# rafaelsoStanford/State_Policy_DiffusionModel

Hardware: AMD Instinct MI355X
Metric: denoise-steps/sec (B=4096, horizon=32) (higher is better)
Workload: dtype f32 (split-fp16 MFMA operands, fp32 accumulate)

## Files before the change

state_policy_diffusionmodel_amd/csrc/device_utils.h:

```cpp
#pragma once
#include <hip/hip_runtime.h>
#include "kernels.h"

namespace spdm {

__device__ __forceinline__ void sample_mean_rstd(const StatsRef& st, int b, float& mean, float& rstd) {
    const long long r0 = (long long)b * st.HW;
    const int first = (int)(r0 / st.m_tile);
    const int last = (int)((r0 + st.HW - 1) / st.m_tile);
    const int n = (last - first + 1) * st.n_tiles;
    const double* p = st.p + (size_t)b * st.slots * 2;
    double s1 = 0.0, s2 = 0.0;
    for (int i = 0; i < n; ++i) { s1 += p[2 * i]; s2 += p[2 * i + 1]; }
    const double m = s1 * st.inv_count;
    double var = s2 * st.inv_count - m * m;
    if (var < 0.0) var = 0.0;
    mean = (float)m;
    rstd = (float)(1.0 / sqrt(var + 1e-5));
}

__device__ __forceinline__ float sum_xor32(float v) {
    const unsigned u = __builtin_bit_cast(unsigned, v);
    const auto r = __builtin_amdgcn_permlane32_swap(u, u, false, false);
    return __builtin_bit_cast(float, (unsigned)r[0]) + __builtin_bit_cast(float, (unsigned)r[1]);
}
__device__ __forceinline__ float max_xor32(float v) {
    const unsigned u = __builtin_bit_cast(unsigned, v);
    const auto r = __builtin_amdgcn_permlane32_swap(u, u, false, false);
    return fmaxf(__builtin_bit_cast(float, (unsigned)r[0]), __builtin_bit_cast(float, (unsigned)r[1]));
}
__device__ __forceinline__ float sum_xor16(float v) {
    const unsigned u = __builtin_bit_cast(unsigned, v);
    const auto r = __builtin_amdgcn_permlane16_swap(u, u, false, false);
    return __builtin_bit_cast(float, (unsigned)r[0]) + __builtin_bit_cast(float, (unsigned)r[1]);
}
__device__ __forceinline__ double sum_xor32_f64(double v) {
    const unsigned long long u = __builtin_bit_cast(unsigned long long, v);
    const unsigned lo = (unsigned)u, hi = (unsigned)(u >> 32);
    const auto rl = __builtin_amdgcn_permlane32_swap(lo, lo, false, false);
    const auto rh = __builtin_amdgcn_permlane32_swap(hi, hi, false, false);
    const double a = __builtin_bit_cast(double, ((unsigned long long)(unsigned)rh[0] << 32) | (unsigned)rl[0]);
    const double b = __builtin_bit_cast(double, ((unsigned long long)(unsigned)rh[1] << 32) | (unsigned)rl[1]);
    return a + b;
}
__device__ __forceinline__ double sum_xor16_f64(double v) {
    const unsigned long long u = __builtin_bit_cast(unsigned long long, v);
    const unsigned lo = (unsigned)u, hi = (unsigned)(u >> 32);
    const auto rl = __builtin_amdgcn_permlane16_swap(lo, lo, false, false);
    const auto rh = __builtin_amdgcn_permlane16_swap(hi, hi, false, false);
    const double a = __builtin_bit_cast(double, ((unsigned long long)(unsigned)rh[0] << 32) | (unsigned)rl[0]);
    const double b = __builtin_bit_cast(double, ((unsigned long long)(unsigned)rh[1] << 32) | (unsigned)rl[1]);
    return a + b;
}

__device__ __forceinline__ void split_pair_f16(float a, float b, unsigned& hi, unsigned& lo) {
    unsigned h;
    float la, lb;
    asm("v_cvt_pk_f16_f32 %0, %1, %2" : "=v"(h) : "v"(a), "v"(b));
    asm("v_fma_mix_f32 %0, %1, -1.0, %2 op_sel:[0,0,0] op_sel_hi:[1,0,0]" : "=v"(la) : "v"(h), "v"(a));
    asm("v_fma_mix_f32 %0, %1, -1.0, %2 op_sel:[1,0,0] op_sel_hi:[1,0,0]" : "=v"(lb) : "v"(h), "v"(b));
    asm("v_cvt_pk_f16_f32 %0, %1, %2" : "=v"(lo) : "v"(la), "v"(lb));
    hi = h;
}

__device__ __forceinline__ double wave_sum_f64(double v) {
#define DPP_ADD64(ctrl_)                                                                                        \
    {                                                                                                           \
        const unsigned long long u_ = __builtin_bit_cast(unsigned long long, v);                                \
        const int lo_ = __builtin_amdgcn_update_dpp(0, (int)(unsigned)u_, ctrl_, 0xf, 0xf, false);             \
        const int hi_ = __builtin_amdgcn_update_dpp(0, (int)(unsigned)(u_ >> 32), ctrl_, 0xf, 0xf, false);     \
        v += __builtin_bit_cast(double, ((unsigned long long)(unsigned)hi_ << 32) | (unsigned long long)(unsigned)lo_); \
    }
    DPP_ADD64(0xB1)
    DPP_ADD64(0x4E)
    DPP_ADD64(0x141)
    DPP_ADD64(0x140)
#undef DPP_ADD64
    v = sum_xor16_f64(v);
    v = sum_xor32_f64(v);
    return v;
}

__device__ __forceinline__ double seg_sum_f64(double v, int seg) {
#define DPP_ADD64(ctrl_)                                                                                        \
    {                                                                                                           \
        const unsigned long long u_ = __builtin_bit_cast(unsigned long long, v);                                \
        const int lo_ = __builtin_amdgcn_update_dpp(0, (int)(unsigned)u_, ctrl_, 0xf, 0xf, false);             \
        const int hi_ = __builtin_amdgcn_update_dpp(0, (int)(unsigned)(u_ >> 32), ctrl_, 0xf, 0xf, false);     \
        v += __builtin_bit_cast(double, ((unsigned long long)(unsigned)hi_ << 32) | (unsigned long long)(unsigned)lo_); \
    }
    if (seg > 1) DPP_ADD64(0xB1)
    if (seg > 2) DPP_ADD64(0x4E)
    if (seg > 4) DPP_ADD64(0x141)
    if (seg > 8) DPP_ADD64(0x140)
#undef DPP_ADD64
    if (seg > 16) v = sum_xor16_f64(v);
    if (seg > 32) v = sum_xor32_f64(v);
    return v;
}

__device__ __forceinline__ void sample_mean_rstd_wave(const StatsRef& st, int b, int lane, float& mean, float& rstd) {
    const long long r0 = (long long)b * st.HW;
    const int first = (int)(r0 / st.m_tile);
    const int last = (int)((r0 + st.HW - 1) / st.m_tile);
    const int n = (last - first + 1) * st.n_tiles;
    if (n <= 8) {
        sample_mean_rstd(st, b, mean, rstd);
        return;
    }
    const double* p = st.p + (size_t)b * st.slots * 2;
    double s1 = 0.0, s2 = 0.0;
// ... 86 lines not shown
```

state_policy_diffusionmodel_amd/csrc/sa_tail.hip:

```cpp
#include <algorithm>
#include <cstdlib>

#include "device_utils.h"

namespace spdm {

namespace {

typedef float tf32x4 __attribute__((ext_vector_type(4)));
typedef float tf32x2 __attribute__((ext_vector_type(2)));
typedef _Float16 tf16x8 __attribute__((ext_vector_type(8)));
typedef _Float16 tf16x2 __attribute__((ext_vector_type(2)));

constexpr float T_ACT_SCALE = 16.0f;
constexpr float T_DESCALE = 1.0f / 2048.0f;
constexpr int T_LDK = 36;
template <int C> struct TailShape {
    static_assert(C == 128 || C == 256, "C = 128 or 256");
    static constexpr int TM = 8192 / C;
    static constexpr int WM = TM / 32, WN = 4 / WM;
    static constexpr int NCH = C / 32;
    static constexpr int TPR = C / 4, RPP = 256 / TPR;
    static constexpr int NP = TM / RPP;
};

struct SaTailArgs {
    const float* o;
    const float* x;
    float* out;
    int M;
    const float *wf_o, *wf_1, *wf_2;
    const float *b_o, *b_1, *b_2, *ln_g, *ln_b;
    const float* ab; int L;
    FilmSpec fs;
};

__device__ __forceinline__ tf32x2 tsplit2_plain(float a, float b) {
    const float xa = a * T_ACT_SCALE, xb = b * T_ACT_SCALE;
    const _Float16 ha = (_Float16)xa, hb = (_Float16)xb;
    const tf16x2 h = {ha, hb};
    const tf16x2 l = {(_Float16)(xa - (float)ha), (_Float16)(xb - (float)hb)};
    return tf32x2{__builtin_bit_cast(float, h), __builtin_bit_cast(float, l)};
}
#define TAIL_SPLIT2 tsplit2
__device__ __forceinline__ tf32x2 tsplit2(float a, float b) {
    unsigned h, l;
    split_pair_f16(a * T_ACT_SCALE, b * T_ACT_SCALE, h, l);
    return tf32x2{__builtin_bit_cast(float, h), __builtin_bit_cast(float, l)};
}
template <int TPR>
__device__ __forceinline__ float trow_sum(float v) {
    static_assert(TPR == 32 || TPR == 64, "rows of 32 or 64 lanes");
    v = sum_xor16(row16_sum_dpp(v));
    if (TPR == 64) v = sum_xor32(v);
    return v;
}

template <int C>
__device__ __forceinline__ void tail_film_fold(tf32x4 (&v)[8], const float* __restrict__ ab, int L, int m0, int M, int cq, int srow0) {
    using S = TailShape<C>;
    if (L % S::TM == 0) {
        const float* ab_ = ab + (size_t)(m0 / L) * 2 * C + cq * 4;
        const tf32x4 A = *reinterpret_cast<const tf32x4*>(ab_), B = *reinterpret_cast<const tf32x4*>(ab_ + C);
#pragma unroll
        for (int i = 0; i < 8; ++i) v[i] = v[i] * A + B;
    } else {
#pragma unroll
        for (int i = 0; i < 8; ++i) {
            const float* ab_ = ab + (size_t)(min(m0 + S::RPP * i + srow0, M - 1) / L) * 2 * C + cq * 4;
            v[i] = v[i] * *reinterpret_cast<const tf32x4*>(ab_) + *reinterpret_cast<const tf32x4*>(ab_ + C);
        }
    }
}

template <int C>
__device__ __forceinline__ void tail_film_rows(const FilmSpec& fs, int L, int m0, int M, int wave, int lane, float* abl) {
    using S = TailShape<C>;
    const int b_first = m0 / L, b_last = (min(m0 + S::TM, M) - 1) / L;
    for (int sidx = wave; sidx <= b_last - b_first; sidx += 4) film_coef_row_wave(fs, b_first + sidx, lane, abl + (size_t)sidx * 2 * C);
}
template <int C>
__device__ __forceinline__ void tail_film_fold_lds(tf32x4 (&v)[8], const float* abl, int L, int m0, int M, int cq, int srow0) {
    using S = TailShape<C>;
    const int b_first = m0 / L;
    if (L % S::TM == 0) {
        const tf32x4 A = *reinterpret_cast<const tf32x4*>(abl + cq * 4), B = *reinterpret_cast<const tf32x4*>(abl + C + cq * 4);
#pragma unroll
        for (int i = 0; i < 8; ++i) v[i] = v[i] * A + B;
    } else {
#pragma unroll
        for (int i = 0; i < 8; ++i) {
            const float* ab_ = abl + (size_t)(min(m0 + S::RPP * i + srow0, M - 1) / L - b_first) * 2 * C + cq * 4;
            v[i] = v[i] * *reinterpret_cast<const tf32x4*>(ab_) + *reinterpret_cast<const tf32x4*>(ab_ + C);
        }
    }
}

#ifdef SPDM_DIAG_TAIL
__device__ unsigned long long g_tail_stamps[64];
#define TAIL_STAMP(k_) if (blockIdx.x == 0 && threadIdx.x == 0) { asm volatile("s_waitcnt vmcnt(0) lgkmcnt(0)" ::: "memory"); g_tail_stamps[(C == 256 ? 16 : 0) + (k_)] = __builtin_amdgcn_s_memrealtime(); }
#else
#define TAIL_STAMP(k_)
#endif

template <int C>
__global__ __launch_bounds__(256, 2) void sa_tail_kernel(const SaTailArgs a) {
    TAIL_STAMP(0)
    using S = TailShape<C>;
    constexpr int T_C = C, T_M = S::TM, NCH = S::NCH, RPP = S::RPP, TPR = S::TPR;
    constexpr int RT = 2, CT = 4;
    constexpr int NP = S::NP;
    extern __shared__ __attribute__((aligned(16))) float smem[];
    const int tid = threadIdx.x, lane = tid & 63;
    const int wave = __builtin_amdgcn_readfirstlane(tid >> 6);
    const int wm = wave / S::WN, wn = wave % S::WN, l16 = lane & 15, kg = lane >> 4;
    const int M = a.M;
    const int m0 = blockIdx.x * T_M;

    float* Abuf = smem;
    float* otile = smem;

    const int c16 = tid % TPR, srow0 = tid / TPR;
    const int aoff0 = (wm * 32 + l16) * T_LDK + kg * 4;

    const size_t wlane = ((size_t)(wn * CT) * 2) * 256 + lane * 4;
    constexpr size_t WCHUNK = (size_t)(C / 16) * 2 * 256;
    tf16x8 fb[2][CT][2], fa[2][2];
#define TAIL_LOAD_B(slot_, w_, kc_)                                                                  \
    {                                                                                                \
        const float* p_ = (w_) + wlane + (size_t)(kc_) * WCHUNK;                                     \
        _Pragma("unroll") for (int c_ = 0; c_ < CT; ++c_) {                                         \
            fb[slot_][c_][0] = *reinterpret_cast<const tf16x8*>(p_ + c_ * 512);                      \
            fb[slot_][c_][1] = *reinterpret_cast<const tf16x8*>(p_ + c_ * 512 + 256);                \
        }                                                                                            \
    }
#define TAIL_LOAD_FA(slot_, kc_, rt_)                                                                \
    {                                                                                                \
        const float* p_ = Abuf + ((kc_) * T_M + (rt_) * 16) * T_LDK + aoff0;                         \
        fa[slot_][0] = *reinterpret_cast<const tf16x8*>(p_);                                         \
        fa[slot_][1] = *reinterpret_cast<const tf16x8*>(p_ + 16);                                    \
    }
#define TAIL_WRITE_SLAB(v_)                                                                          \
    _Pragma("unroll") for (int i_ = 0; i_ < NP; ++i_) {                                             \
        const tf32x2 p0_ = TAIL_SPLIT2(v_[i_].x, v_[i_].y), p1_ = TAIL_SPLIT2(v_[i_].z, v_[i_].w);   \
        float* rowp_ = Abuf + ((c16 >> 3) * T_M + RPP * i_ + srow0) * T_LDK;                         \
        *reinterpret_cast<tf32x2*>(rowp_ + (c16 & 7) * 2) = tf32x2{p0_.x, p1_.x};                    \
        *reinterpret_cast<tf32x2*>(rowp_ + 16 + (c16 & 7) * 2) = tf32x2{p0_.y, p1_.y};               \
    }
#define TAIL_GEMM(w_, wnext_)                                                                        \
    {                                                                                                \
        _Pragma("unroll") for (int rt_ = 0; rt_ < RT; ++rt_)                                        \
            _Pragma("unroll") for (int ct_ = 0; ct_ < CT; ++ct_) acc[rt_][ct_] = tf32x4{0.f, 0.f, 0.f, 0.f}; \
        TAIL_LOAD_FA(0, 0, 0)                                                                        \
        _Pragma("unroll") for (int kc = 0; kc < NCH; ++kc) {                                        \
            if (kc + 1 < NCH) { TAIL_LOAD_B((kc + 1) & 1, w_, kc + 1) } else { TAIL_LOAD_B(0, wnext_, 0) } \
            _Pragma("unroll") for (int rt = 0; rt < RT; ++rt) {                                     \
                if (rt + 1 < RT) { TAIL_LOAD_FA((rt + 1) & 1, kc, rt + 1) }                          \
                else if (kc + 1 < NCH) { TAIL_LOAD_FA(0, kc + 1, 0) }                                \
                __builtin_amdgcn_sched_barrier(0);                                                   \
                _Pragma("unroll") for (int c = 0; c < CT; ++c)                                      \
                    acc[rt][c] = __builtin_amdgcn_mfma_f32_16x16x32_f16(fa[rt & 1][0], fb[kc & 1][c][0], acc[rt][c], 0, 0, 0); \
                _Pragma("unroll") for (int c = 0; c < CT; ++c)                                      \
                    acc[rt][c] = __builtin_amdgcn_mfma_f32_16x16x32_f16(fa[rt & 1][0], fb[kc & 1][c][1], acc[rt][c], 0, 0, 0); \
                _Pragma("unroll") for (int c = 0; c < CT; ++c)                                      \
                    acc[rt][c] = __builtin_amdgcn_mfma_f32_16x16x32_f16(fa[rt & 1][1], fb[kc & 1][c][0], acc[rt][c], 0, 0, 0); \
                __builtin_amdgcn_sched_barrier(0);                                                   \
            }                                                                                        \
        }                                                                                            \
    }
#define TAIL_ACC_TO_TILE()                                                                           \
    {                                                                                                \
        __syncthreads();                                                                             \
        _Pragma("unroll") for (int rt_ = 0; rt_ < RT; ++rt_)                                        \
            _Pragma("unroll") for (int ct_ = 0; ct_ < CT; ++ct_) {                                  \
                const int col_ = wn * 64 + ct_ * 16 + l16;                                           \
                _Pragma("unroll") for (int j_ = 0; j_ < 4; ++j_)                                    \
                    otile[(wm * 32 + rt_ * 16 + 4 * kg + j_) * T_C + col_] = acc[rt_][ct_][j_] * T_DESCALE; \
            }                                                                                        \
        __syncthreads();                                                                             \
    }

    TAIL_LOAD_B(0, a.wf_o, 0)
    float* abl = smem + NCH * T_M * T_LDK;
    const tf32x4 bo = *reinterpret_cast<const tf32x4*>(a.b_o + c16 * 4);
    const tf32x4 g4 = *reinterpret_cast<const tf32x4*>(a.ln_g + c16 * 4);
// ... 150 lines not shown
        if (a.ab != nullptr) tail_film_fold<C>(v, a.ab, a.L, m0, M, c16, srow0);
        if (a.fs.on) {
            float* abl = smem + NCH * T_M * T_LDK;
            tail_film_rows<C>(a.fs, a.L, m0, M, wave, lane, abl);
            __syncthreads();
            tail_film_fold_lds<C>(v, abl, a.L, m0, M, c16, srow0);
        }
        float part[NP];
#pragma unroll
        for (int i = 0; i < NP; ++i) part[i] = (v[i].x + v[i].y) + (v[i].z + v[i].w);
#pragma unroll
        for (int i = 0; i < NP; ++i) part[i] = row16_sum_dpp(part[i]);
#pragma unroll
        for (int i = 0; i < NP; ++i) part[i] = sum_xor16(part[i]);
        if (TPR == 64) {
#pragma unroll
            for (int i = 0; i < NP; ++i) part[i] = sum_xor32(part[i]);
        }
#pragma unroll
        for (int i = 0; i < NP; ++i) {
            const float mean = part[i] * (1.0f / (float)C);
            const tf32x4 t = v[i];
            const tf32x4 d = {t.x - mean, t.y - mean, t.z - mean, t.w - mean};
            v[i] = d;
            part[i] = (d.x * d.x + d.y * d.y) + (d.z * d.z + d.w * d.w);
        }
#pragma unroll
        for (int i = 0; i < NP; ++i) part[i] = row16_sum_dpp(part[i]);
#pragma unroll
        for (int i = 0; i < NP; ++i) part[i] = sum_xor16(part[i]);
        if (TPR == 64) {
#pragma unroll
            for (int i = 0; i < NP; ++i) part[i] = sum_xor32(part[i]);
        }
#pragma unroll
        for (int i = 0; i < NP; ++i) {
            const float rstd = __builtin_amdgcn_rsqf(part[i] * (1.0f / (float)C) + 1e-5f);
            const tf32x4 d = v[i];
            v[i] = tf32x4{d.x * rstd * g4.x + b4.x, d.y * rstd * g4.y + b4.y, d.z * rstd * g4.z + b4.z, d.w * rstd * g4.w + b4.w};
        }
    }
    TAIL_WRITE_SLAB(v)
    __syncthreads();
    for (int g = g_lo; g < g_hi; ++g) {
        const float* wg = a.wf + (size_t)g * WPROD;
        const float* wnext = a.wf + (size_t)(g < 2 ? g + 1 : g) * WPROD;
        const tf32x4 bi = *reinterpret_cast<const tf32x4*>(a.b_in + g * T_C + c16 * 4);
        TAIL_GEMM(wg, wnext)
        {
            float* ot = smem + NCH * T_M * T_LDK;
            if (g > g_lo) __syncthreads();
#pragma unroll
            for (int rt_ = 0; rt_ < RT; ++rt_)
#pragma unroll
                for (int ct_ = 0; ct_ < CT; ++ct_) {
                    const int col_ = wn * 64 + ct_ * 16 + l16;
#pragma unroll
                    for (int j_ = 0; j_ < 4; ++j_)
                        ot[(wm * 32 + rt_ * 16 + 4 * kg + j_) * T_C + col_] = acc[rt_][ct_][j_] * T_DESCALE;
                }
            __syncthreads();
#pragma unroll
            for (int i = 0; i < NP; ++i) {
                const int r = RPP * i + srow0;
                if (m0 + r < M) {
                    tf32x4 t = *reinterpret_cast<const tf32x4*>(ot + r * T_C + c16 * 4);
                    t += bi;
                    *reinterpret_cast<tf32x4*>(a.qkv + (size_t)(m0 + r) * (3 * T_C) + g * T_C + c16 * 4) = t;
                }
            }
        }
    }
    (void)otile;
}

struct SaHeadArgs {
    const float* x; float* att; int M;
    const float* wf;
    const float *b_in, *ln_g, *ln_b;
    const float* ab; int L;
    FilmSpec fs;
};

__device__ __forceinline__ float row16_max_dpp(float v) {
#define DPP_MAX(ctrl_) v = fmaxf(v, __builtin_bit_cast(float, __builtin_amdgcn_update_dpp(0, __builtin_bit_cast(int, v), ctrl_, 0xf, 0xf, false)));
    DPP_MAX(0xB1) DPP_MAX(0x4E) DPP_MAX(0x141) DPP_MAX(0x140)
#undef DPP_MAX
    return v;
}
__device__ __forceinline__ float head_exp_neg(float x) {
    const float t = x * 1.44269504f;
    const float tl = __fmaf_rn(x, 1.44269504f, -t) + x * 1.925963033e-8f;
    return __builtin_amdgcn_exp2f(t) * (1.0f + tl * 0.69314718f);
}

#undef TAIL_SPLIT2
#define TAIL_SPLIT2 tsplit2_plain
template <int C>
__global__ __launch_bounds__(256, 2) void sa_head_kernel(const SaHeadArgs a) {
    using S = TailShape<C>;
    constexpr int T_C = C, T_M = S::TM, NCH = S::NCH, RPP = S::RPP, TPR = S::TPR;
    constexpr int NP = S::NP;
    constexpr int D = C / 4;
    constexpr int QROW = 2 * D + 8;
    constexpr int VROW = 2 * T_M + 8;
    constexpr int NKT = T_M / 16;
    constexpr int NDT = D / 16;
    static_assert(T_M * VROW <= 2 * T_M * QROW, "P aliases the q / k tiles");
    extern __shared__ __attribute__((aligned(16))) float smem[];
    const int tid = threadIdx.x, lane = tid & 63;
    const int wave = __builtin_amdgcn_readfirstlane(tid >> 6);
    const int l16 = lane & 15, kg = lane >> 4;
    const int M = a.M, L = a.L;
    const int m0 = blockIdx.x * T_M;
    float* Abuf = smem;
    _Float16* Qs = reinterpret_cast<_Float16*>(smem + NCH * T_M * T_LDK);
    _Float16* Ks = Qs + T_M * QROW;
    _Float16* Vt = Ks + T_M * QROW;
    _Float16* Ps = Qs;
    const int c16 = tid % TPR, srow0 = tid / TPR;

    {
        tf32x4 v[NP];
        const tf32x4 g4 = *reinterpret_cast<const tf32x4*>(a.ln_g + c16 * 4);
        const tf32x4 b4 = *reinterpret_cast<const tf32x4*>(a.ln_b + c16 * 4);
#pragma unroll
        for (int i = 0; i < NP; ++i) {
            const int row = min(m0 + RPP * i + srow0, M - 1);
            v[i] = *reinterpret_cast<const tf32x4*>(a.x + (size_t)row * T_C + c16 * 4);
        }
        if (a.ab != nullptr) tail_film_fold<C>(v, a.ab, a.L, m0, M, c16, srow0);
        if (a.fs.on) {
            float* abl = reinterpret_cast<float*>(Qs);
            tail_film_rows<C>(a.fs, a.L, m0, M, wave, lane, abl);
            __syncthreads();
            tail_film_fold_lds<C>(v, abl, a.L, m0, M, c16, srow0);
            __syncthreads();
        }
        float part[NP];
#pragma unroll
        for (int i = 0; i < NP; ++i) part[i] = (v[i].x + v[i].y) + (v[i].z + v[i].w);
#pragma unroll
        for (int i = 0; i < NP; ++i) part[i] = trow_sum<TPR>(part[i]);
#pragma unroll
        for (int i = 0; i < NP; ++i) {
            const float mean = part[i] * (1.0f / (float)C);
            const tf32x4 t = v[i];
            const tf32x4 d = {t.x - mean, t.y - mean, t.z - mean, t.w - mean};
            v[i] = d;
            part[i] = (d.x * d.x + d.y * d.y) + (d.z * d.z + d.w * d.w);
        }
#pragma unroll
        for (int i = 0; i < NP; ++i) part[i] = trow_sum<TPR>(part[i]);
#pragma unroll
        for (int i = 0; i < NP; ++i) {
            const float rstd = __builtin_amdgcn_rsqf(part[i] * (1.0f / (float)C) + 1e-5f);
            const tf32x4 d = v[i];
            v[i] = tf32x4{d.x * rstd * g4.x + b4.x, d.y * rstd * g4.y + b4.y, d.z * rstd * g4.z + b4.z, d.w * rstd * g4.w + b4.w};
        }
        TAIL_WRITE_SLAB(v)
    }
    __syncthreads();

    const int rtw = (C == 128) ? wave : (wave >> 1);
    const int cpw = (C == 128) ? 0 : (wave & 1);
    const bool attn_wave = wave < NKT;
    const float qscale = (D == 32) ? 0.17677669529663687f : 0.125f;
    constexpr size_t WCHUNK = (size_t)(3 * C / 16) * 2 * 256;

    tf16x8 fbw[2][2][2];
#define HEAD_WPTR(h_, g_) (a.wf + ((size_t)((g_) * (C / 16) + (h_) * (D / 16) + cpw * 2) * 2) * 256 + lane * 4)
#define HEAD_LOAD_W(slot_, wp_, kc_)                                                                 \
    _Pragma("unroll") for (int ct_ = 0; ct_ < 2; ++ct_) {                                           \
        fbw[slot_][ct_][0] = *reinterpret_cast<const tf16x8*>((wp_) + (size_t)(kc_) * WCHUNK + ct_ * 512);        \
        fbw[slot_][ct_][1] = *reinterpret_cast<const tf16x8*>((wp_) + (size_t)(kc_) * WCHUNK + ct_ * 512 + 256);  \
    }
    HEAD_LOAD_W(0, HEAD_WPTR(0, 0), 0)
    for (int h = 0; h < 4; ++h) {
#pragma unroll
        for (int g = 0; g < 3; ++g) {
            tf32x4 acc[2] = {tf32x4{0.f, 0.f, 0.f, 0.f}, tf32x4{0.f, 0.f, 0.f, 0.f}};
            const float* wp = HEAD_WPTR(h, g);
            const float* wnext = (g < 2) ? HEAD_WPTR(h, g + 1) : HEAD_WPTR(min(h + 1, 3), 0);
#pragma unroll
            for (int kc = 0; kc < NCH; ++kc) {
                if (kc + 1 < NCH) { HEAD_LOAD_W((kc + 1) & 1, wp, kc + 1) } else { HEAD_LOAD_W(0, wnext, 0) }
                const float* ap = Abuf + (kc * T_M + rtw * 16 + l16) * T_LDK + kg * 4;
                const tf16x8 a_h = *reinterpret_cast<const tf16x8*>(ap), a_l = *reinterpret_cast<const tf16x8*>(ap + 16);
#pragma unroll
                for (int ct = 0; ct < 2; ++ct) {
                    acc[ct] = __builtin_amdgcn_mfma_f32_16x16x32_f16(a_h, fbw[kc & 1][ct][0], acc[ct], 0, 0, 0);
                    acc[ct] = __builtin_amdgcn_mfma_f32_16x16x32_f16(a_h, fbw[kc & 1][ct][1], acc[ct], 0, 0, 0);
                    acc[ct] = __builtin_amdgcn_mfma_f32_16x16x32_f16(a_l, fbw[kc & 1][ct][0], acc[ct], 0, 0, 0);
                }
            }
#pragma unroll
            for (int ct = 0; ct < 2; ++ct) {
                const int col = cpw * 32 + ct * 16 + l16;
                const float bias = a.b_in[g * T_C + h * D + col];
#pragma unroll
                for (int j = 0; j < 4; ++j) {
                    const int row = rtw * 16 + 4 * kg + j;
                    float val = acc[ct][j] * T_DESCALE + bias;
                    if (g == 0) val *= qscale;
                    const float xs = val * T_ACT_SCALE;
                    const _Float16 hi = (_Float16)xs, lo = (_Float16)(xs - (float)hi);
                    if (g == 2) { Vt[col * VROW + row] = hi; Vt[col * VROW + T_M + row] = lo; }
                    else { _Float16* X = (g == 0) ? Qs : Ks; X[row * QROW + col] = hi; X[row * QROW + D + col] = lo; }
                }
            }
        }
        __syncthreads();

        tf32x4 sc[NKT];
#pragma unroll
        for (int kt = 0; kt < NKT; ++kt) sc[kt] = tf32x4{0.f, 0.f, 0.f, 0.f};
        if (attn_wave) {
#pragma unroll
            for (int ks = 0; ks < D / 32; ++ks) {
                const _Float16* qp = Qs + (wave * 16 + l16) * QROW + 32 * ks + 8 * kg;
                const tf16x8 q_h = *reinterpret_cast<const tf16x8*>(qp), q_l = *reinterpret_cast<const tf16x8*>(qp + D);
#pragma unroll
                for (int kt = 0; kt < NKT; ++kt) {
                    const _Float16* kp = Ks + (kt * 16 + l16) * QROW + 32 * ks + 8 * kg;
                    const tf16x8 k_h = *reinterpret_cast<const tf16x8*>(kp), k_l = *reinterpret_cast<const tf16x8*>(kp + D);
                    sc[kt] = __builtin_amdgcn_mfma_f32_16x16x32_f16(q_h, k_h, sc[kt], 0, 0, 0);
                    sc[kt] = __builtin_amdgcn_mfma_f32_16x16x32_f16(q_h, k_l, sc[kt], 0, 0, 0);
                    sc[kt] = __builtin_amdgcn_mfma_f32_16x16x32_f16(q_l, k_h, sc[kt], 0, 0, 0);
                }
            }
        }
        __syncthreads();

        if (attn_wave) {
#pragma unroll
            for (int j = 0; j < 4; ++j) {
                const int row = wave * 16 + 4 * kg + j;
                const int smp = row / L;
                float s[NKT];
                float mx = -3.0e38f;
#pragma unroll
                for (int kt = 0; kt < NKT; ++kt) {
                    const bool own = ((kt * 16 + l16) / L) == smp;
                    s[kt] = own ? sc[kt][j] * (1.0f / 256.0f) : -3.0e38f;
                    mx = fmaxf(mx, s[kt]);
                }
                mx = row16_max_dpp(mx);
                float sum = 0.f;
#pragma unroll
                for (int kt = 0; kt < NKT; ++kt) {
                    s[kt] = (s[kt] > -1.0e38f) ? head_exp_neg(s[kt] - mx) : 0.f;
                    sum += s[kt];
                }
                sum = row16_sum_dpp(sum);
                const float inv = 1024.0f / sum;
#pragma unroll
                for (int kt = 0; kt < NKT; ++kt) {
                    const float ps = s[kt] * inv;
                    const _Float16 hi = (_Float16)ps, lo = (_Float16)(ps - (float)hi);
                    Ps[row * VROW + kt * 16 + l16] = hi;
                    Ps[row * VROW + T_M + kt * 16 + l16] = lo;
                }
            }
        }
        __syncthreads();

        if (attn_wave) {
            tf32x4 o[NDT];
#pragma unroll
            for (int dt = 0; dt < NDT; ++dt) o[dt] = tf32x4{0.f, 0.f, 0.f, 0.f};
#pragma unroll
            for (int ks = 0; ks < T_M / 32; ++ks) {
                const _Float16* pp = Ps + (wave * 16 + l16) * VROW + 32 * ks + 8 * kg;
                const tf16x8 p_h = *reinterpret_cast<const tf16x8*>(pp), p_l = *reinterpret_cast<const tf16x8*>(pp + T_M);
#pragma unroll
                for (int dt = 0; dt < NDT; ++dt) {
                    const _Float16* vp = Vt + (dt * 16 + l16) * VROW + 32 * ks + 8 * kg;
                    const tf16x8 v_h = *reinterpret_cast<const tf16x8*>(vp), v_l = *reinterpret_cast<const tf16x8*>(vp + T_M);
                    o[dt] = __builtin_amdgcn_mfma_f32_16x16x32_f16(p_h, v_h, o[dt], 0, 0, 0);
                    o[dt] = __builtin_amdgcn_mfma_f32_16x16x32_f16(p_h, v_l, o[dt], 0, 0, 0);
                    o[dt] = __builtin_amdgcn_mfma_f32_16x16x32_f16(p_l, v_h, o[dt], 0, 0, 0);
                }
            }
#pragma unroll
            for (int dt = 0; dt < NDT; ++dt)
#pragma unroll
                for (int j = 0; j < 4; ++j) {
                    const int row = m0 + wave * 16 + 4 * kg + j;
                    if (row < M) a.att[(size_t)row * T_C + h * D + dt * 16 + l16] = o[dt][j] * (1.0f / 16384.0f);
                }
        }
        __syncthreads();
    }
#undef TAIL_LOAD_B
#undef TAIL_LOAD_FA
#undef TAIL_WRITE_SLAB
#undef TAIL_GEMM
#undef TAIL_ACC_TO_TILE
}

}

#ifdef SPDM_DIAG_TAIL
extern "C" int spdm_debug_tail_stamps(unsigned long long* out64) {
    return hipMemcpyFromSymbol(out64, HIP_SYMBOL(g_tail_stamps), sizeof(unsigned long long) * 64) == hipSuccess ? 0 : -1;
}
#endif

bool sa_tail_supported(int C, unsigned sw) { return (C == 128 || C == 256) && !(sw & SW_NO_SA_TAIL); }

static int film_rows_cap(int TM, int L) { return (TM + L - 2) / L + 1; }
bool sa_tail_film_local(int C, int L) {
    if (!(C == 128 || C == 256) || L < 1) return false;
    return (size_t)film_rows_cap(8192 / C, L) * 2 * C * sizeof(float) <= (size_t)24 * 1024;
}

hipError_t launch_sa_tail(int C, const float* o, const float* x, float* out, int rows, const float* wf_o, const float* wf_1,
                          const float* wf_2, const float* b_o, const float* b_1, const float* b_2, const float* ln_g,
                          const float* ln_b, const float* ab, int L, hipStream_t s, const FilmSpec* fs) {
    if (fs && (ab || L <= 0 || !sa_tail_film_local(C, L) || fs->C != C)) return hipErrorInvalidValue;
    if (rows <= 0 || (ab && L <= 0) || !o || !x || !out || !wf_o || !wf_1 || !wf_2 || !b_o || !b_1 || !b_2 || !ln_g || !ln_b)
        return hipErrorInvalidValue;
    if (C != 128 && C != 256) return hipErrorInvalidValue;
    SaTailArgs a{};
    a.o = o; a.x = x; a.out = out; a.M = rows;
    a.wf_o = wf_o; a.wf_1 = wf_1; a.wf_2 = wf_2;
    a.b_o = b_o; a.b_1 = b_1; a.b_2 = b_2; a.ln_g = ln_g; a.ln_b = ln_b; a.ab = ab; a.L = L;
    if (fs) { a.fs = *fs; a.fs.on = 1; }
    const int TM = 8192 / C;
    const size_t lds = (size_t)(C / 32) * TM * T_LDK * sizeof(float)
                       + (fs ? (size_t)film_rows_cap(TM, L) * 2 * C * sizeof(float) : 0);
    if (C == 128) hipLaunchKernelGGL(sa_tail_kernel<128>, dim3((rows + TM - 1) / TM), dim3(256), lds, s, a);
    else hipLaunchKernelGGL(sa_tail_kernel<256>, dim3((rows + TM - 1) / TM), dim3(256), lds, s, a);
    return hipGetLastError();
}

bool sa_head_supported(int C, int L, unsigned sw) {
    return (C == 128 || C == 256) && L >= 1 && (8192 / C) % L == 0 && !(sw & (SW_NO_SA_TAIL | SW_NO_SA_HEAD));
}

hipError_t launch_sa_head(int C, const float* x, float* att, int rows, const float* wf_in, const float* b_in, const float* ln_g,
                          const float* ln_b, const float* ab, int L, hipStream_t s, const FilmSpec* fs) {
    if (rows <= 0 || !x || !att || !wf_in || !b_in || !ln_g || !ln_b || !sa_head_supported(C, L, 0) || rows % L != 0) return hipErrorInvalidValue;
    if (fs && (ab || !sa_tail_film_local(C, L) || fs->C != C)) return hipErrorInvalidValue;
    SaHeadArgs a{};
    a.x = x; a.att = att; a.M = rows; a.wf = wf_in; a.b_in = b_in; a.ln_g = ln_g; a.ln_b = ln_b; a.ab = ab; a.L = L;
    if (fs) { a.fs = *fs; a.fs.on = 1; }
    const int TM = 8192 / C, D = C / 4;
    const size_t lds = (size_t)(C / 32) * TM * T_LDK * sizeof(float) + ((size_t)2 * TM * (2 * D + 8) + (size_t)D * (2 * TM + 8)) * sizeof(_Float16);
    if (fs && (size_t)film_rows_cap(TM, L) * 2 * C * sizeof(float) > ((size_t)2 * TM * (2 * D + 8) + (size_t)D * (2 * TM + 8)) * sizeof(_Float16)) return hipErrorInvalidValue;
    const void* kern = C == 128 ? reinterpret_cast<const void*>(sa_head_kernel<128>) : reinterpret_cast<const void*>(sa_head_kernel<256>);
    if (hipError_t e = allow_full_lds(kern); e != hipSuccess) return e;
    const int tiles = (rows + TM - 1) / TM;
    if (C == 128) hipLaunchKernelGGL(sa_head_kernel<128>, dim3(tiles), dim3(256), lds, s, a);
    else hipLaunchKernelGGL(sa_head_kernel<256>, dim3(tiles), dim3(256), lds, s, a);
    return hipGetLastError();
}

hipError_t launch_sa_qkv(int C, const float* x, float* qkv, int rows, const float* wf_in, const float* b_in, const float* ln_g,
                         const float* ln_b, const float* ab, int L, hipStream_t s, const FilmSpec* fs) {
    if (fs && (ab || L <= 0 || !sa_tail_film_local(C, L) || fs->C != C)) return hipErrorInvalidValue;
    if (rows <= 0 || (ab && L <= 0) || !x || !qkv || !wf_in || !b_in || !ln_g || !ln_b) return hipErrorInvalidValue;
    if (C != 128 && C != 256) return hipErrorInvalidValue;
    SaQkvArgs a{};
    a.x = x; a.qkv = qkv; a.M = rows; a.wf = wf_in; a.b_in = b_in; a.ln_g = ln_g; a.ln_b = ln_b; a.ab = ab; a.L = L;
    if (fs) { a.fs = *fs; a.fs.on = 1; }
    const int TM = 8192 / C;
    const size_t lds = (size_t)((C / 32) * TM * T_LDK + TM * C) * sizeof(float);
    const void* kern = C == 128 ? reinterpret_cast<const void*>(sa_qkv_kernel<128>) : reinterpret_cast<const void*>(sa_qkv_kernel<256>);
    if (hipError_t e = allow_full_lds(kern); e != hipSuccess) return e;
    const int tiles = (rows + TM - 1) / TM;
    const int gy = (tiles < spdm_tune(15, 512)) ? 3 : 1;
    if (C == 128) hipLaunchKernelGGL(sa_qkv_kernel<128>, dim3(tiles, gy), dim3(256), lds, s, a);
    else hipLaunchKernelGGL(sa_qkv_kernel<256>, dim3(tiles, gy), dim3(256), lds, s, a);
    return hipGetLastError();
}
// ... 3 lines not shown
```

Baseline: 532,300.

## Restructure attention head kernel: register-resident softmax, block-diagonal skip, deeper weight ring

Rewrites the per-head loop of the self-attention head kernel. Weight fragments now stream through a ring of RD register slots that carries across heads. Activation fragments are loaded once per block instead of per projection. Q/K/V projections are computed together, with transposed MFMA operands so results come out in the layout the next step needs, and are written to LDS as vector stores. QK^T and PV run on all waves, and key tiles outside the wave's sample (the block-diagonal mask) are skipped. Softmax stays in registers, uses permlane swaps, and feeds PV directly without an LDS round trip for P, removing two barriers per head. Costs are higher register pressure from the ring and fragment caches, which may hurt occupancy, plus optional diagnostic timestamps.

```diff
diff --git a/state_policy_diffusionmodel_amd/csrc/device_utils.h b/state_policy_diffusionmodel_amd/csrc/device_utils.h
--- a/state_policy_diffusionmodel_amd/csrc/device_utils.h
+++ b/state_policy_diffusionmodel_amd/csrc/device_utils.h
@@ -27,6 +27,11 @@
 __device__ __forceinline__ float max_xor32(float v) {
     const unsigned u = __builtin_bit_cast(unsigned, v);
     const auto r = __builtin_amdgcn_permlane32_swap(u, u, false, false);
+    return fmaxf(__builtin_bit_cast(float, (unsigned)r[0]), __builtin_bit_cast(float, (unsigned)r[1]));
+}
+__device__ __forceinline__ float max_xor16(float v) {
+    const unsigned u = __builtin_bit_cast(unsigned, v);
+    const auto r = __builtin_amdgcn_permlane16_swap(u, u, false, false);
     return fmaxf(__builtin_bit_cast(float, (unsigned)r[0]), __builtin_bit_cast(float, (unsigned)r[1]));
 }
 __device__ __forceinline__ float sum_xor16(float v) {
diff --git a/state_policy_diffusionmodel_amd/csrc/sa_tail.hip b/state_policy_diffusionmodel_amd/csrc/sa_tail.hip
--- a/state_policy_diffusionmodel_amd/csrc/sa_tail.hip
+++ b/state_policy_diffusionmodel_amd/csrc/sa_tail.hip
@@ -101,6 +101,11 @@
 #define TAIL_STAMP(k_) if (blockIdx.x == 0 && threadIdx.x == 0) { asm volatile("s_waitcnt vmcnt(0) lgkmcnt(0)" ::: "memory"); g_tail_stamps[(C == 256 ? 16 : 0) + (k_)] = __builtin_amdgcn_s_memrealtime(); }
 #else
 #define TAIL_STAMP(k_)
+#endif
+#ifdef SPDM_DIAG_TAIL
+#define HEAD_STAMP(k_) if (blockIdx.x == 0 && threadIdx.x == 0) { asm volatile("s_waitcnt vmcnt(0) lgkmcnt(0)" ::: "memory"); g_tail_stamps[(C == 256 ? 48 : 32) + (k_)] = __builtin_amdgcn_s_memrealtime(); }
+#else
+#define HEAD_STAMP(k_)
 #endif
 
 template <int C>
@@ -417,12 +422,6 @@
     FilmSpec fs;
 };
 
-__device__ __forceinline__ float row16_max_dpp(float v) {
-#define DPP_MAX(ctrl_) v = fmaxf(v, __builtin_bit_cast(float, __builtin_amdgcn_update_dpp(0, __builtin_bit_cast(int, v), ctrl_, 0xf, 0xf, false)));
-    DPP_MAX(0xB1) DPP_MAX(0x4E) DPP_MAX(0x141) DPP_MAX(0x140)
-#undef DPP_MAX
-    return v;
-}
 __device__ __forceinline__ float head_exp_neg(float x) {
     const float t = x * 1.44269504f;
     const float tl = __fmaf_rn(x, 1.44269504f, -t) + x * 1.925963033e-8f;
@@ -431,6 +430,15 @@
 
 #undef TAIL_SPLIT2
 #define TAIL_SPLIT2 tsplit2_plain
+typedef unsigned tu32x2 __attribute__((ext_vector_type(2)));
+typedef unsigned tu32x4 __attribute__((ext_vector_type(4)));
+#ifndef SPDM_HEAD_RD128
+#define SPDM_HEAD_RD128 4
+#endif
+#ifndef SPDM_HEAD_RD256
+#define SPDM_HEAD_RD256 4
+#endif
+
 template <int C>
 __global__ __launch_bounds__(256, 2) void sa_head_kernel(const SaHeadArgs a) {
     using S = TailShape<C>;
@@ -440,20 +448,40 @@
     constexpr int QROW = 2 * D + 8;
     constexpr int VROW = 2 * T_M + 8;
     constexpr int NKT = T_M / 16;
-    constexpr int NDT = D / 16;
-    static_assert(T_M * VROW <= 2 * T_M * QROW, "P aliases the q / k tiles");
+    constexpr int NST = 3 * NCH;
+    constexpr int RD = (C == 128) ? SPDM_HEAD_RD128 : SPDM_HEAD_RD256;
+    static_assert(NST % RD == 0, "the ring keeps its slot numbering across the head loop's back edge");
     extern __shared__ __attribute__((aligned(16))) float smem[];
     const int tid = threadIdx.x, lane = tid & 63;
     const int wave = __builtin_amdgcn_readfirstlane(tid >> 6);
     const int l16 = lane & 15, kg = lane >> 4;
-    const int M = a.M, L = a.L;
+    const int M = a.M;
+    const int lgL = 31 - __builtin_clz(a.L);
     const int m0 = blockIdx.x * T_M;
     float* Abuf = smem;
     _Float16* Qs = reinterpret_cast<_Float16*>(smem + NCH * T_M * T_LDK);
     _Float16* Ks = Qs + T_M * QROW;
     _Float16* Vt = Ks + T_M * QROW;
-    _Float16* Ps = Qs;
     const int c16 = tid % TPR, srow0 = tid / TPR;
+    HEAD_STAMP(0)
+
+    const int rtw = (C == 128) ? wave : (wave >> 1);
+    const int cpw = (C == 128) ? 0 : (wave & 1);
+    const float qscale = (D == 32) ? 0.17677669529663687f : 0.125f;
+    constexpr size_t WCHUNK = (size_t)(3 * C / 16) * 2 * 256;
+
+    tf16x8 fbw[RD][2][2];
+    const float* wbase = a.wf + ((size_t)(cpw * 2) * 2) * 256 + lane * 4;
+#define HEAD_LOAD_W(slot_, wh_, u_)                                                                  \
+    {                                                                                                \
+        const float* wp_ = (wh_) + (size_t)((u_) / NCH) * (C / 16) * 512 + (size_t)((u_) % NCH) * WCHUNK; \
+        _Pragma("unroll") for (int ct_ = 0; ct_ < 2; ++ct_) {                                       \
+            fbw[slot_][ct_][0] = *reinterpret_cast<const tf16x8*>(wp_ + ct_ * 512);                  \
+            fbw[slot_][ct_][1] = *reinterpret_cast<const tf16x8*>(wp_ + ct_ * 512 + 256);            \
+        }                                                                                            \
+    }
+#pragma unroll
+    for (int u = 0; u < RD; ++u) HEAD_LOAD_W(u, wbase, u)
 
     {
         tf32x4 v[NP];
@@ -496,137 +524,195 @@
         TAIL_WRITE_SLAB(v)
     }
     __syncthreads();
-
-    const int rtw = (C == 128) ? wave : (wave >> 1);
-    const int cpw = (C == 128) ? 0 : (wave & 1);
-    const bool attn_wave = wave < NKT;
-    const float qscale = (D == 32) ? 0.17677669529663687f : 0.125f;
-    constexpr size_t WCHUNK = (size_t)(3 * C / 16) * 2 * 256;
-
-    tf16x8 fbw[2][2][2];
-#define HEAD_WPTR(h_, g_) (a.wf + ((size_t)((g_) * (C / 16) + (h_) * (D / 16) + cpw * 2) * 2) * 256 + lane * 4)
-#define HEAD_LOAD_W(slot_, wp_, kc_)                                                                 \
-    _Pragma("unroll") for (int ct_ = 0; ct_ < 2; ++ct_) {                                           \
-        fbw[slot_][ct_][0] = *reinterpret_cast<const tf16x8*>((wp_) + (size_t)(kc_) * WCHUNK + ct_ * 512);        \
-        fbw[slot_][ct_][1] = *reinterpret_cast<const tf16x8*>((wp_) + (size_t)(kc_) * WCHUNK + ct_ * 512 + 256);  \
-    }
-    HEAD_LOAD_W(0, HEAD_WPTR(0, 0), 0)
+    tf16x8 af[NCH][2];
+#pragma unroll
+    for (int kc = 0; kc < NCH; ++kc) {
+        const float* ap = Abuf + (kc * T_M + rtw * 16 + l16) * T_LDK + kg * 4;
+        af[kc][0] = *reinterpret_cast<const tf16x8*>(ap);
+        af[kc][1] = *reinterpret_cast<const tf16x8*>(ap + 16);
+    }
+    HEAD_STAMP(1)
+
+    unsigned need = 0;
+#pragma unroll
+    for (int kt = 0; kt < NKT; ++kt) need |= (((16 * kt) >> lgL) == ((16 * rtw) >> lgL)) ? (1u << kt) : 0u;
+    need = __builtin_amdgcn_readfirstlane(need);
+    const int qsmp = (rtw * 16 + l16) >> lgL;
+
     for (int h = 0; h < 4; ++h) {
+        const float* wh = wbase + (size_t)h * (D / 16) * 512;
+        const float* whn = wbase + (size_t)min(h + 1, 3) * (D / 16) * 512;
+        tf32x4 bqk[2][2];
+        float bv[2];
+#pragma unroll
+        for (int ct = 0; ct < 2; ++ct) {
+            bqk[0][ct] = *reinterpret_cast<const tf32x4*>(a.b_in + h * D + cpw * 32 + ct * 16 + 4 * kg);
+            bqk[1][ct] = *reinterpret_cast<const tf32x4*>(a.b_in + T_C + h * D + cpw * 32 + ct * 16 + 4 * kg);
+            bv[ct] = a.b_in[2 * T_C + h * D + cpw * 32 + ct * 16 + l16];
+        }
+        tf32x4 acc[3][2];
 #pragma unroll
         for (int g = 0; g < 3; ++g) {
-            tf32x4 acc[2] = {tf32x4{0.f, 0.f, 0.f, 0.f}, tf32x4{0.f, 0.f, 0.f, 0.f}};
-            const float* wp = HEAD_WPTR(h, g);
-            const float* wnext = (g < 2) ? HEAD_WPTR(h, g + 1) : HEAD_WPTR(min(h + 1, 3), 0);
+            acc[g][0] = tf32x4{0.f, 0.f, 0.f, 0.f};
+            acc[g][1] = tf32x4{0.f, 0.f, 0.f, 0.f};
 #pragma unroll
             for (int kc = 0; kc < NCH; ++kc) {
-                if (kc + 1 < NCH) { HEAD_LOAD_W((kc + 1) & 1, wp, kc + 1) } else { HEAD_LOAD_W(0, wnext, 0) }
-                const float* ap = Abuf + (kc * T_M + rtw * 16 + l16) * T_LDK + kg * 4;
-                const tf16x8 a_h = *reinterpret_cast<const tf16x8*>(ap), a_l = *reinterpret_cast<const tf16x8*>(ap + 16);
+                const int u = g * NCH + kc, sl = u % RD;
+                const tf16x8 a_h = af[kc][0], a_l = af[kc][1];
 #pragma unroll
                 for (int ct = 0; ct < 2; ++ct) {
-                    acc[ct] = __builtin_amdgcn_mfma_f32_16x16x32_f16(a_h, fbw[kc & 1][ct][0], acc[ct], 0, 0, 0);
-                    acc[ct] = __builtin_amdgcn_mfma_f32_16x16x32_f16(a_h, fbw[kc & 1][ct][1], acc[ct], 0, 0, 0);
-                    acc[ct] = __builtin_amdgcn_mfma_f32_16x16x32_f16(a_l, fbw[kc & 1][ct][0], acc[ct], 0, 0, 0);
-                }
-            }
+                    if (g < 2) {
+                        acc[g][ct] = __builtin_amdgcn_mfma_f32_16x16x32_f16(fbw[sl][ct][0], a_h, acc[g][ct], 0, 0, 0);
+                        acc[g][ct] = __builtin_amdgcn_mfma_f32_16x16x32_f16(fbw[sl][ct][1], a_h, acc[g][ct], 0, 0, 0);
+                        acc[g][ct] = __builtin_amdgcn_mfma_f32_16x16x32_f16(fbw[sl][ct][0], a_l, acc[g][ct], 0, 0, 0);
+                    } else {
+                        acc[g][ct] = __builtin_amdgcn_mfma_f32_16x16x32_f16(a_h, fbw[sl][ct][0], acc[g][ct], 0, 0, 0);
+                        acc[g][ct] = __builtin_amdgcn_mfma_f32_16x16x32_f16(a_h, fbw[sl][ct][1], acc[g][ct], 0, 0, 0);
+                        acc[g][ct] = __builtin_amdgcn_mfma_f32_16x16x32_f16(a_l, fbw[sl][ct][0], acc[g][ct], 0, 0, 0);
+                    }
+                }
+                if (u + RD < NST) { HEAD_LOAD_W(sl, wh, u + RD) } else { HEAD_LOAD_W(sl, whn, u + RD - NST) }
+                __builtin_amdgcn_sched_barrier(0);
+            }
+            if (h == 0) { HEAD_STAMP(2 + 2 * g) HEAD_STAMP(3 + 2 * g) }
+        }
+        __syncthreads();
+
+#pragma unroll
+        for (int g = 0; g < 2; ++g) {
+            _Float16* X = (g == 0) ? Qs : Ks;
 #pragma unroll
             for (int ct = 0; ct < 2; ++ct) {
-                const int col = cpw * 32 + ct * 16 + l16;
-                const float bias = a.b_in[g * T_C + h * D + col];
+                float val[4];
 #pragma unroll
                 for (int j = 0; j < 4; ++j) {
-                    const int row = rtw * 16 + 4 * kg + j;
-                    float val = acc[ct][j] * T_DESCALE + bias;
-                    if (g == 0) val *= qscale;
-                    const float xs = val * T_ACT_SCALE;
-                    const _Float16 hi = (_Float16)xs, lo = (_Float16)(xs - (float)hi);
-                    if (g == 2) { Vt[col * VROW + row] = hi; Vt[col * VROW + T_M + row] = lo; }
-                    else { _Float16* X = (g == 0) ? Qs : Ks; X[row * QROW + col] = hi; X[row * QROW + D + col] = lo; }
-                }
-            }
-        }
+                    val[j] = acc[g][ct][j] * T_DESCALE + bqk[g][ct][j];
+                    if (g == 0) val[j] *= qscale;
+                    val[j] *= T_ACT_SCALE;
+                }
+                unsigned h0, l0, h1, l1;
+                split_pair_f16(val[0], val[1], h0, l0);
+                split_pair_f16(val[2], val[3], h1, l1);
+                const tu32x2 hi = {h0, h1}, lo = {l0, l1};
+                _Float16* xp = X + (rtw * 16 + l16) * QROW + cpw * 32 + ct * 16 + 4 * kg;
+                *reinterpret_cast<tu32x2*>(xp) = hi;
+                *reinterpret_cast<tu32x2*>(xp + D) = lo;
+            }
+        }
+#pragma unroll
+        for (int ct = 0; ct < 2; ++ct) {
+            float val[4];
+#pragma unroll
+            for (int j = 0; j < 4; ++j) val[j] = (acc[2][ct][j] * T_DESCALE + bv[ct]) * T_ACT_SCALE;
+            unsigned h0, l0, h1, l1;
+            split_pair_f16(val[0], val[1], h0, l0);
+            split_pair_f16(val[2], val[3], h1, l1);
+            const tu32x2 hi = {h0, h1}, lo = {l0, l1};
+            _Float16* vp = Vt + (cpw * 32 + ct * 16 + l16) * VROW + 32 * (rtw >> 1) + 8 * kg + 4 * (rtw & 1);
+            *reinterpret_cast<tu32x2*>(vp) = hi;
+            *reinterpret_cast<tu32x2*>(vp + T_M) = lo;
+        }
+        if (h == 0) { HEAD_STAMP(7) }
         __syncthreads();
+        if (h == 0) { HEAD_STAMP(8) }
 
         tf32x4 sc[NKT];
-#pragma unroll
-        for (int kt = 0; kt < NKT; ++kt) sc[kt] = tf32x4{0.f, 0.f, 0.f, 0.f};
-        if (attn_wave) {
+        {
+            tf16x8 q_h[D / 32], q_l[D / 32];
 #pragma unroll
             for (int ks = 0; ks < D / 32; ++ks) {
-                const _Float16* qp = Qs + (wave * 16 + l16) * QROW + 32 * ks + 8 * kg;
-                const tf16x8 q_h = *reinterpret_cast<const tf16x8*>(qp), q_l = *reinterpret_cast<const tf16x8*>(qp + D);
-#pragma unroll
-                for (int kt = 0; kt < NKT; ++kt) {
-                    const _Float16* kp = Ks + (kt * 16 + l16) * QROW + 32 * ks + 8 * kg;
-                    const tf16x8 k_h = *reinterpret_cast<const tf16x8*>(kp), k_l = *reinterpret_cast<const tf16x8*>(kp + D);
-                    sc[kt] = __builtin_amdgcn_mfma_f32_16x16x32_f16(q_h, k_h, sc[kt], 0, 0, 0);
-                    sc[kt] = __builtin_amdgcn_mfma_f32_16x16x32_f16(q_h, k_l, sc[kt], 0, 0, 0);
-                    sc[kt] = __builtin_amdgcn_mfma_f32_16x16x32_f16(q_l, k_h, sc[kt], 0, 0, 0);
-                }
-            }
-        }
-        __syncthreads();
-
-        if (attn_wave) {
-#pragma unroll
-            for (int j = 0; j < 4; ++j) {
-                const int row = wave * 16 + 4 * kg + j;
-                const int smp = row / L;
-                float s[NKT];
-                float mx = -3.0e38f;
-#pragma unroll
-                for (int kt = 0; kt < NKT; ++kt) {
-                    const bool own = ((kt * 16 + l16) / L) == smp;
-                    s[kt] = own ? sc[kt][j] * (1.0f / 256.0f) : -3.0e38f;
-                    mx = fmaxf(mx, s[kt]);
-                }
-                mx = row16_max_dpp(mx);
-                float sum = 0.f;
-#pragma unroll
-                for (int kt = 0; kt < NKT; ++kt) {
-                    s[kt] = (s[kt] > -1.0e38f) ? head_exp_neg(s[kt] - mx) : 0.f;
-                    sum += s[kt];
-                }
-                sum = row16_sum_dpp(sum);
-                const float inv = 1024.0f / sum;
-#pragma unroll
-                for (int kt = 0; kt < NKT; ++kt) {
-                    const float ps = s[kt] * inv;
-                    const _Float16 hi = (_Float16)ps, lo = (_Float16)(ps - (float)hi);
-                    Ps[row * VROW + kt * 16 + l16] = hi;
-                    Ps[row * VROW + T_M + kt * 16 + l16] = lo;
-                }
-            }
-        }
-        __syncthreads();
-
-        if (attn_wave) {
-            tf32x4 o[NDT];
-#pragma unroll
-            for (int dt = 0; dt < NDT; ++dt) o[dt] = tf32x4{0.f, 0.f, 0.f, 0.f};
-#pragma unroll
-            for (int ks = 0; ks < T_M / 32; ++ks) {
-                const _Float16* pp = Ps + (wave * 16 + l16) * VROW + 32 * ks + 8 * kg;
-                const tf16x8 p_h = *reinterpret_cast<const tf16x8*>(pp), p_l = *reinterpret_cast<const tf16x8*>(pp + T_M);
-#pragma unroll
-                for (int dt = 0; dt < NDT; ++dt) {
-                    const _Float16* vp = Vt + (dt * 16 + l16) * VROW + 32 * ks + 8 * kg;
-                    const tf16x8 v_h = *reinterpret_cast<const tf16x8*>(vp), v_l = *reinterpret_cast<const tf16x8*>(vp + T_M);
-                    o[dt] = __builtin_amdgcn_mfma_f32_16x16x32_f16(p_h, v_h, o[dt], 0, 0, 0);
-                    o[dt] = __builtin_amdgcn_mfma_f32_16x16x32_f16(p_h, v_l, o[dt], 0, 0, 0);
-                    o[dt] = __builtin_amdgcn_mfma_f32_16x16x32_f16(p_l, v_h, o[dt], 0, 0, 0);
-                }
-            }
-#pragma unroll
-            for (int dt = 0; dt < NDT; ++dt)
-#pragma unroll
-                for (int j = 0; j < 4; ++j) {
-                    const int row = m0 + wave * 16 + 4 * kg + j;
-                    if (row < M) a.att[(size_t)row * T_C + h * D + dt * 16 + l16] = o[dt][j] * (1.0f / 16384.0f);
-                }
-        }
-        __syncthreads();
-    }
+                const _Float16* qp = Qs + (rtw * 16 + l16) * QROW + 32 * ks + 8 * kg;
+                q_h[ks] = *reinterpret_cast<const tf16x8*>(qp);
+                q_l[ks] = *reinterpret_cast<const tf16x8*>(qp + D);
+            }
+#pragma unroll
+            for (int kt = 0; kt < NKT; ++kt) {
+                sc[kt] = tf32x4{0.f, 0.f, 0.f, 0.f};
+                if (need & (1u << kt)) {
+#pragma unroll
+                    for (int ks = 0; ks < D / 32; ++ks) {
+                        const _Float16* kp = Ks + (kt * 16 + l16) * QROW + 32 * ks + 8 * kg;
+                        const tf16x8 k_h = *reinterpret_cast<const tf16x8*>(kp), k_l = *reinterpret_cast<const tf16x8*>(kp + D);
+                        sc[kt] = __builtin_amdgcn_mfma_f32_16x16x32_f16(k_h, q_h[ks], sc[kt], 0, 0, 0);
+                        sc[kt] = __builtin_amdgcn_mfma_f32_16x16x32_f16(k_l, q_h[ks], sc[kt], 0, 0, 0);
+                        sc[kt] = __builtin_amdgcn_mfma_f32_16x16x32_f16(k_h, q_l[ks], sc[kt], 0, 0, 0);
+                    }
+                }
+            }
+        }
+        if (h == 0) { HEAD_STAMP(9) HEAD_STAMP(10) }
+
+        tf16x8 p_h[NKT / 2], p_l[NKT / 2];
+        {
+            float mx = -3.0e38f;
+#pragma unroll
+            for (int kt = 0; kt < NKT; ++kt) {
+                if (need & (1u << kt)) {
+#pragma unroll
+                    for (int j = 0; j < 4; ++j) {
+                        const bool own = ((kt * 16 + 4 * kg + j) >> lgL) == qsmp;
+                        sc[kt][j] = own ? sc[kt][j] * (1.0f / 256.0f) : -3.0e38f;
+                        mx = fmaxf(mx, sc[kt][j]);
+                    }
+                }
+            }
+            mx = max_xor32(max_xor16(mx));
+            float sum = 0.f;
+#pragma unroll
+            for (int kt = 0; kt < NKT; ++kt) {
+                if (need & (1u << kt)) {
+#pragma unroll
+                    for (int j = 0; j < 4; ++j) {
+                        sc[kt][j] = (sc[kt][j] > -1.0e38f) ? head_exp_neg(sc[kt][j] - mx) : 0.f;
+                        sum += sc[kt][j];
+                    }
+                }
+            }
+            sum = sum_xor32(sum_xor16(sum));
+            const float inv = 1024.0f / sum;
+#pragma unroll
+            for (int s = 0; s < NKT / 2; ++s) {
+                unsigned ph[4] = {0u, 0u, 0u, 0u}, pl[4] = {0u, 0u, 0u, 0u};
+                if (need & (1u << (2 * s))) {
+                    split_pair_f16(sc[2 * s][0] * inv, sc[2 * s][1] * inv, ph[0], pl[0]);
+                    split_pair_f16(sc[2 * s][2] * inv, sc[2 * s][3] * inv, ph[1], pl[1]);
+                }
+                if (need & (2u << (2 * s))) {
+                    split_pair_f16(sc[2 * s + 1][0] * inv, sc[2 * s + 1][1] * inv, ph[2], pl[2]);
+                    split_pair_f16(sc[2 * s + 1][2] * inv, sc[2 * s + 1][3] * inv, ph[3], pl[3]);
+                }
+                p_h[s] = __builtin_bit_cast(tf16x8, tu32x4{ph[0], ph[1], ph[2], ph[3]});
+                p_l[s] = __builtin_bit_cast(tf16x8, tu32x4{pl[0], pl[1], pl[2], pl[3]});
+            }
+        }
+        if (h == 0) { HEAD_STAMP(11) HEAD_STAMP(12) }
+
+        {
+            tf32x4 o[2] = {tf32x4{0.f, 0.f, 0.f, 0.f}, tf32x4{0.f, 0.f, 0.f, 0.f}};
+#pragma unroll
+            for (int s = 0; s < NKT / 2; ++s) {
+                if (need & (3u << (2 * s))) {
+#pragma unroll
+                    for (int dt = 0; dt < 2; ++dt) {
+                        const _Float16* vp = Vt + (cpw * 32 + dt * 16 + l16) * VROW + 32 * s + 8 * kg;
+                        const tf16x8 v_h = *reinterpret_cast<const tf16x8*>(vp), v_l = *reinterpret_cast<const tf16x8*>(vp + T_M);
+                        o[dt] = __builtin_amdgcn_mfma_f32_16x16x32_f16(v_h, p_h[s], o[dt], 0, 0, 0);
+                        o[dt] = __builtin_amdgcn_mfma_f32_16x16x32_f16(v_l, p_h[s], o[dt], 0, 0, 0);
+                        o[dt] = __builtin_amdgcn_mfma_f32_16x16x32_f16(v_h, p_l[s], o[dt], 0, 0, 0);
+                    }
+                }
+            }
+            const int row = m0 + rtw * 16 + l16;
+            if (row < M) {
+#pragma unroll
+                for (int dt = 0; dt < 2; ++dt)
+                    *reinterpret_cast<tf32x4*>(a.att + (size_t)row * T_C + h * D + cpw * 32 + dt * 16 + 4 * kg) = o[dt] * (1.0f / 16384.0f);
+            }
+        }
+        if (h == 0) { HEAD_STAMP(13) HEAD_STAMP(14) }
+    }
+    HEAD_STAMP(15)
+#undef HEAD_LOAD_W
 #undef TAIL_LOAD_B
 #undef TAIL_LOAD_FA
 #undef TAIL_WRITE_SLAB
```

Result: no change. 535,200, median of 6 (+0.6%).
